# leospeidel/Colate

Hardware: NVIDIA B200
Metric: pair_site_evals_per_s (higher is better)
Workload: dtype f64

## Files before the change

### colate_b200/csrc/kernels_em.cu

```cuda
#include <cooperative_groups.h>

#include "device.cuh"
#include "glibc_math.cuh"

#include <cstring>

namespace cg = cooperative_groups;

namespace colate {

constexpr int EM_THREADS = 416;
constexpr int EM_TASKS = 384;

__global__ void __launch_bounds__(256)
k_bootstrap(int num_blocks, const int32_t* __restrict__ weights, const double* __restrict__ blk,
            double age, const double* __restrict__ age_bin, double* __restrict__ counts, int norm_1e3)
{
  __shared__ double S[NBINS], N[NBINS], SE[NBINS], NE[NBINS], F[NBINS];
  __shared__ double s_fcount, s_normf;
  const int r = blockIdx.x;
  const int32_t* w = weights + (size_t)r * num_blocks;
  int bin_start = 0;
  while (bin_start < NBINS - 1 && age_bin[bin_start] <= age) bin_start++;
  for (int b = threadIdx.x; b < NBINS; b += blockDim.x) {
// ... 377 lines not shown
        }
        __syncthreads();
        if (tid < cw) {
          double acc = 0.0;
#pragma unroll 10
          for (int j = 0; j < n_task; j++) acc += stage[j * cw + tid];
          const int col = c0 + tid;
          for (int r = 0; r < csize; r++) {
            if (col < E) cluster.map_shared_rank(tn, r)[col] = acc;
            else if (col < 2 * E) cluster.map_shared_rank(td, r)[col - E] = acc;
            else cluster.map_shared_rank(&ll_new, r)[0] = acc;
          }
        }
        __syncthreads();
      }
      cluster.sync();
      if (tid == 0) { prev_s = ll_s; ll_s = ll_new; }
    } else {
      double acc = 0.0;
      int buf = 0;
      for (int col = tid + EM_THREADS; col <= 2 * E; col += EM_THREADS) (col < 2 * E ? tn[col] : ll_new) = 0.0;
      for (int i = tid; i < min(TJ, n_task) * RS; i += blockDim.x) stage[i] = __ldcg(M + i);
      __syncthreads();
      for (int j0 = 0; j0 < n_task; j0 += TJ) {
        const int nj = min(TJ, n_task - j0);
        const int j1 = j0 + TJ, nn = (j1 < n_task) ? min(TJ, n_task - j1) : 0;
        double pre[9];
        const double* src = M + (size_t)j1 * RS;
#pragma unroll
        for (int u = 0; u < 9; u++) { const int i = tid + u * EM_THREADS; pre[u] = (i < nn * RS) ? __ldcg(src + i) : 0.0; }
        if (tid <= 2 * E) {
          const double* col = stage + (size_t)buf * EM_STAGE_DOUBLES + tid;
          for (int j = 0; j < nj; j++) acc += col[(size_t)j * RS];
        }
        for (int c2 = tid + EM_THREADS; c2 <= 2 * E; c2 += EM_THREADS) {
          const double* col = stage + (size_t)buf * EM_STAGE_DOUBLES + c2;
          double& a2 = c2 < 2 * E ? tn[c2] : ll_new;
          double s = a2;
          for (int j = 0; j < nj; j++) s += col[(size_t)j * RS];
          a2 = s;
        }
        double* dst = stage + (size_t)(buf ^ 1) * EM_STAGE_DOUBLES;
#pragma unroll
        for (int u = 0; u < 9; u++) { const int i = tid + u * EM_THREADS; if (i < nn * RS) dst[i] = pre[u]; }
        __syncthreads();
        buf ^= 1;
      }
      if (tid < E) tn[tid] = acc;
      else if (tid < 2 * E) td[tid - E] = acc;
      else if (tid == 2 * E) { prev_s = ll_s; ll_s = acc; }
      if (2 * E >= EM_THREADS && tid == 2 * E % EM_THREADS) { prev_s = ll_s; ll_s = ll_new; }
    }
    __syncthreads();
    if (prof) { t1 = clock64(); tp[4] += t1 - t0; t0 = t1; }
    for (int e = tid; e < E; e += blockDim.x) {
      const double n_ = tn[e], d_ = td[e];
      double r = rate[e];
      if (n_ != 0 && d_ != 0) { r = n_ / d_; r = (r < 5e-9) ? 5e-9 : r; }
      cand[e] = r;
    }
    __syncthreads();
    for (int e = tid; e < E; e += blockDim.x) {
      int s = e;
      while (s >= 0 && tn[s] == 0) s--;
      rate[e] = (s >= 0) ? cand[s] : 0.0;
    }
    if (tid == 0 && (ll_s / prev_s > 1.0 - 1e-7) && (iter > 1000)) stop_flag = 1;
    __syncthreads();
    if (prof) { t1 = clock64(); tp[5] += t1 - t0; t0 = t1; }
    if (stop_flag) break;
  }
  if (prof && tid == 0) for (int i = 0; i < 6; i++) prof[i] = tp[i];
  if (prof && tid == 384) prof[6] = tp[1];
  if (prof && tid == 192 + 8 * crank + 1) prof[7] = tp[1];
  if (crank == 0) {
    for (int e = tid; e < E; e += blockDim.x) rates_out[(size_t)rep * E + e] = rate[e];
    if (tid == 0) { iters_out[rep] = iter; ll_out[rep] = ll_s; }
  }
}

constexpr int EMS_THREADS = 640;
constexpr int EMS_FOLD_WARPS = 12;
constexpr int EMS_TLMAX = 96;

__device__ __forceinline__ uint32_t em_smem_u32(const void* p) { return (uint32_t)__cvta_generic_to_shared(p); }
__device__ __forceinline__ uint32_t em_mapa(uint32_t saddr, int rank)
{
  uint32_t r;
  asm volatile("mapa.shared::cluster.u32 %0, %1, %2;" : "=r"(r) : "r"(saddr), "r"(rank));
  return r;
}
__device__ __forceinline__ void em_st_async(uint32_t raddr, double v, uint32_t rbar)
{
  asm volatile("st.async.weak.shared::cluster.mbarrier::complete_tx::bytes.b64 [%0], %1, [%2];" ::"r"(raddr),
               "l"(__double_as_longlong(v)), "r"(rbar) : "memory");
}
__device__ __forceinline__ void em_mbar_init(uint64_t* bar, int count)
{
  asm volatile("mbarrier.init.shared::cta.b64 [%0], %1;" ::"r"(em_smem_u32(bar)), "r"(count) : "memory");
}
__device__ __forceinline__ void em_mbar_arm(uint64_t* bar, uint32_t bytes)
{
  asm volatile("mbarrier.arrive.expect_tx.shared::cta.b64 _, [%0], %1;" ::"r"(em_smem_u32(bar)), "r"(bytes) : "memory");
}
__device__ __forceinline__ bool em_mbar_wait(uint64_t* bar, uint32_t parity)
{
  const long long t0 = clock64();
  for (;;) {
    uint32_t done;
    asm volatile(
        "{\n\t.reg .pred p;\n\t"
        "mbarrier.try_wait.parity.acquire.cluster.shared::cta.b64 p, [%1], %2;\n\t"
        "selp.u32 %0, 1, 0, p;\n\t}" : "=r"(done) : "r"(em_smem_u32(bar)), "r"(parity) : "memory");
    if (done) return true;
    if (clock64() - t0 > 4000000000ll) return false;
  }
}
__device__ __forceinline__ void named_bar_sync(int id, int n) { asm volatile("bar.sync %0, %1;" ::"r"(id), "r"(n) : "memory"); }
__device__ __forceinline__ void named_bar_arrive(int id, int n) { asm volatile("bar.arrive %0, %1;" ::"r"(id), "r"(n) : "memory"); }

__global__ void __launch_bounds__(EMS_THREADS, 1)
k_em_split(int E, const double* __restrict__ epochs, const double* __restrict__ rates_init,
           const double* __restrict__ age_bin_g, const double* __restrict__ counts, int max_iter,
           const uint64_t* __restrict__ exp_tab_g, const uint64_t* __restrict__ log_tab_g, double* scratch,
           double* __restrict__ rates_out, int32_t* __restrict__ iters_out, double* __restrict__ ll_out, long long* prof_g)
{
  cg::cluster_group cluster = cg::this_cluster();
  const int crank = (int)cluster.block_rank(), csize = (int)cluster.num_blocks();
  const int rep = blockIdx.x / csize;
  const int n_task = 2 * NBINS, ncol = 2 * E + 1, RS = 2 * E + 2;
  const int CW = (ncol + csize - 1) / csize;
  const int nbl = (NBINS + csize - 1) / csize;
  const int ntl = 2 * nbl;

  extern __shared__ double sm[];
  double* ep = sm;
  double* rate = ep + E;
  double* Lam = rate + E;
  double* A = Lam + E;
  double* B = A + E;
  double* PL = B + E;
  double* tn = PL + E + 1;
  double* td = tn + E;
  double* cand = td + E;
  double* prod = cand + E;
  double* raw = prod + E;
  double* integ_s = raw + (size_t)ntl * E * 2;
  double* colbuf = integ_s + (size_t)ntl * E;
  uint64_t* etab = (uint64_t*)(colbuf + (size_t)n_task * CW);
  uint64_t* ltab = etab + 256;
  __shared__ int stop_flag;
  __shared__ double ll_s, prev_s, ll_new;
  __shared__ __align__(8) uint64_t bar_rows, bar_tot;
  __shared__ double h_t[EMS_TLMAX], h_cnt[EMS_TLMAX], h_nc[EMS_TLMAX], h_numt[EMS_TLMAX], h_dent[EMS_TLMAX], h_logl[EMS_TLMAX];
  __shared__ int h_et[EMS_TLMAX], h_good[EMS_TLMAX];

  const int tid = threadIdx.x, warp = tid >> 5, lane = tid & 31;
  const uint32_t magicE = E > 1 ? 0xffffffffu / (uint32_t)E + 1u : 0u, magicCW = CW > 1 ? 0xffffffffu / (uint32_t)CW + 1u : 0u;
  auto divE = [&](int i) { return magicE ? (int)__umulhi((uint32_t)i, magicE) : i; };
  auto divCW = [&](int c) { return magicCW ? (int)__umulhi((uint32_t)c, magicCW) : c; };
  for (int e = tid; e < E; e += blockDim.x) { ep[e] = epochs[e]; rate[e] = rates_init[e]; }
  for (int i = tid; i < 256; i += blockDim.x) { etab[i] = exp_tab_g[i]; ltab[i] = log_tab_g[i]; }
  if (tid == 0) {
    stop_flag = 0; ll_s = neg_inf();
    em_mbar_init(&bar_rows, 1); em_mbar_init(&bar_tot, 1);
    asm volatile("fence.mbarrier_init.release.cluster;" ::: "memory");
  }
  const int n_active = __syncthreads_count(tid < n_task && counts[(size_t)rep * 2 * NBINS + tid] > 0);
  const int my_cw = max(0, min(ncol, crank * CW + CW) - crank * CW);
  const uint32_t bytes_rows = (uint32_t)n_active * my_cw * 8, bytes_tot = (uint32_t)ncol * 8;
  const uint32_t colbuf_s = em_smem_u32(colbuf), tn_s = em_smem_u32(tn), td_s = em_smem_u32(td), ll_sa = em_smem_u32(&ll_new);
  const uint32_t bar_rows_s = em_smem_u32(&bar_rows), bar_tot_s = em_smem_u32(&bar_tot);
  if (tid < ntl) {
    const int b = (tid >> 1) * csize + crank, type = tid & 1;
    double t = 0.0, cnt = 0.0;
    if (b < NBINS) { t = age_bin_g[b]; cnt = counts[(size_t)rep * 2 * NBINS + (type ? NBINS : 0) + b]; }
    h_t[tid] = t;
    h_cnt[tid] = cnt > 0 ? cnt : 0.0;
    h_et[tid] = tint_k(E, ep, t) - 1;
    h_good[tid] = 0; h_nc[tid] = 0.0; h_numt[tid] = 0.0; h_dent[tid] = 0.0; h_logl[tid] = 0.0;
  }
  for (int i = tid; i < n_task * CW; i += blockDim.x) colbuf[i] = 0.0;
  EmCtx c{E, ep, rate, A, B, Lam, glm::Tables{etab, ltab}};
  long long* prof = prof_g ? prof_g + (size_t)blockIdx.x * 16 : nullptr;
  long long tp[16] = {0, 0, 0, 0, 0, 0, 0, 0, 0, 0, 0, 0, 0, 0, 0, 0};
  cluster.sync();

  int iter = 0;
  for (; iter < max_iter; iter++) {
    long long t0 = prof ? clock64() : 0, t1;
    if (tid == 0) { em_mbar_arm(&bar_rows, bytes_rows); em_mbar_arm(&bar_tot, bytes_tot); }
    for (int e = tid + 1; e < E; e += blockDim.x) prod[e] = rate[e - 1] * (ep[e] - ep[e - 1]);
    __syncthreads();
    for (int e = tid; e < E; e += blockDim.x) {
      double l = 0.0;
      for (int i = 1; i <= e; i++) l = l + prod[i];
      Lam[e] = l;
    }
    __syncthreads();
    const int ft0 = (E + 31) & ~31;
    if (tid < E) em_A(E, ep, rate, Lam, tid, A, c.T);
    else if (tid >= ft0 && tid < ft0 + nbl && h_cnt[2 * (tid - ft0) + 1] > 0) {
      const int l = 2 * (tid - ft0) + 1, et = h_et[l], k = et + 1;
      const double t = h_t[l], r = rate[et];
      const double c1 = Lam[et] + r * (t - ep[et]);
      const double c2 = c1 + r * (t - t);
      double num_t;
      if (et != E - 1) {
        const double c3 = c2 + r * (ep[k] - t);
        num_t = (r > 0) ? lme(-c2, -c3, c.T) : neg_inf();
      } else num_t = -c2;
      h_numt[l] = num_t;
    }
    __syncthreads();
    if (prof) { t1 = clock64(); tp[0] += t1 - t0; t0 = t1; }
    if (warp < EMS_FOLD_WARPS) {
      const int fpw = (nbl + EMS_FOLD_WARPS - 1) / EMS_FOLD_WARPS;
      const int f = warp * fpw + lane, l = 2 * f + 1;
      if (lane < fpw && f < nbl && h_cnt[l] > 0) {
        double nc = h_numt[l];
        const int et = h_et[l];
        if (et != E - 1) {
          double v = A[et + 1];
          for (int e = et + 1; e < E; e++) {
            const double vn = A[min(e + 1, E - 1)];
            nc = lse(nc, v, c.T);
            v = vn;
          }
        }
        const bool good = !bad(nc);
        h_nc[l] = nc; h_good[l] = good ? 1 : 0; h_logl[l] = h_cnt[l] * (good ? nc : 0.0);
      }
    } else if (warp == EMS_FOLD_WARPS) {
      if (lane == 0) {
        double nc = A[0], v = A[min(1, E - 1)];
        PL[0] = 1.0;
        PL[1] = nc;
        for (int e = 1; e < E; e++) {
          const double vn = A[min(e + 1, E - 1)];
          if (nc == 1.0) nc = v; else nc = lse(nc, v, c.T);
          PL[e + 1] = nc;
          v = vn;
        }
      }
      named_bar_sync(1, EMS_THREADS - EMS_FOLD_WARPS * 32);
      for (int j = lane; j < nbl; j += 32) {
        const int l = 2 * j;
        if (h_cnt[l] > 0) {
          const double pl = PL[h_et[l]], num_t = h_numt[l];
          const double nc = (pl == 1.0) ? num_t : lse(pl, num_t, c.T);
          const bool good = !bad(nc);
          h_nc[l] = nc; h_good[l] = good ? 1 : 0; h_logl[l] = h_cnt[l] * (good ? nc : 0.0);
        }
      }
    } else {
      const int q = tid - (EMS_FOLD_WARPS + 1) * 32;
      if (q < E) em_B(E, ep, rate, Lam, q, B, c.T);
      else if (q < E + nbl) {
        const int l = 2 * (q - E) + 1;
        if (h_cnt[l] > 0) {
          const int et = h_et[l], k = et + 1;
          const double t = h_t[l], r = rate[et], inv = 1.0 / r;
          const double c1 = Lam[et] + r * (t - ep[et]);
          const double c2 = c1 + r * (t - t);
          double den_t;
          if (et != E - 1) {
            const double c3 = c2 + r * (ep[k] - t);
            den_t = (r > 0) ? glm::log((t + inv) - (ep[k] + inv) * glm::exp(-c3 + c2, c.T), c.T) - c2 : neg_inf();
          } else den_t = glm::log(t + inv, c.T) - c2;
          h_dent[l] = den_t;
        }
      } else if (q < E + 2 * nbl) {
        const int l = 2 * (q - E - nbl);
        if (h_cnt[l] > 0) {
          double num_t, den_t;
          shared_special(c, h_t[l], h_et[l], num_t, den_t);
          h_numt[l] = num_t; h_dent[l] = den_t;
        }
      }
      named_bar_arrive(1, EMS_THREADS - EMS_FOLD_WARPS * 32);
    }
    __syncthreads();
    if (prof) { t1 = clock64(); tp[1] += t1 - t0; t0 = t1; }
    auto raw_term = [&](int i, int which) {
      const int l = divE(i), e = i - l * E, et = h_et[l];
      const bool sh = (l & 1) == 0;
      const int lim = (E - 1 < et + 1) ? E - 1 : et + 1;
      const bool need = h_good[l] && (sh ? (e < lim || (e == E - 1 && et == E - 1)) : (e >= et));
      const bool own = sh ? !(e < et) : (e == et);
      if (need) {
        const double x = (which == 0 ? (own ? h_numt[l] : A[e]) : (own ? h_dent[l] : B[e])) - h_nc[l];
        raw[2 * i + which] = exp_fast(x, c.T);
      }
    };
    for (int i = tid; i < ntl * E; i += blockDim.x) raw_term(i, 0);
    __syncthreads();
    if (prof) { t1 = clock64(); tp[2] += t1 - t0; t0 = t1; }
    const int iw = ((ntl + 31) >> 5) * 32;
    if (tid >= iw) {
      for (int i = tid - iw; i < ntl * E; i += blockDim.x - iw) raw_term(i, 1);
    } else if (tid < ntl && h_good[tid]) {
      const int et = h_et[tid];
      const int lo = (tid & 1) ? et : 0;
      const int hi = (tid & 1) ? E - 1 : ((E - 1 < et + 1) ? E - 1 : et + 1);
      double integ = 1.0;
      const double* __restrict__ rw = raw + (size_t)tid * E * 2;
      double* __restrict__ out = integ_s + tid * E;
      for (int e0 = 0; e0 < E; e0 += 8) {
        double nb[8];
#pragma unroll
        for (int u = 0; u < 8; u++) nb[u] = (e0 + u >= lo && e0 + u < hi) ? rw[2 * (e0 + u)] : 0.0;
#pragma unroll
        for (int u = 0; u < 8; u++) {
          integ = (integ > 0.0) ? integ - nb[u] : 0.0;
          if (e0 + u < E) out[e0 + u] = integ;
        }
      }
    }
    __syncthreads();
    if (prof) { t1 = clock64(); tp[8] += t1 - t0; t0 = t1; }
    for (int i = tid; i < ntl * E; i += blockDim.x) {
      const int l = divE(i), e = i - l * E;
      const double cnt = h_cnt[l];
      if (cnt > 0) {
        const int et = h_et[l];
        double ne = 0.0, de = 0.0;
        if (h_good[l]) {
          const double integ = integ_s[i];
          if ((l & 1) == 0) {
            const int lim = (E - 1 < et + 1) ? E - 1 : et + 1;
            if (e < lim) {
              ne = raw[2 * i];
              de = raw[2 * i + 1];
              de += -ep[e] * ne + (ep[e + 1] - ep[e]) * integ;
              if (de < 0.0) de = 0.0;
            } else if (e == E - 1 && et == E - 1) {
              ne = raw[2 * i];
              de = raw[2 * i + 1];
              de -= ep[e] * ne;
              if (de < 0.0) de = 0.0;
            }
          } else {
            if (e < et) {
              de = ep[e + 1] - ep[e];
            } else {
              ne = raw[2 * i];
              if (e < E - 1) {
                de = raw[2 * i + 1];
                de += -ep[e] * ne + (ep[e + 1] - ep[e]) * integ;
              } else {
                de = raw[2 * i + 1];
                de -= ep[e] * ne;
              }
              if (de < 0.0) de = 0.0;
            }
          }
        }
        const int tk = 2 * ((l >> 1) * csize + crank) + (l & 1);
        const int r1 = divCW(e), r2 = divCW(E + e);
        em_st_async(em_mapa(colbuf_s, r1) + 8u * (tk * CW + (e - r1 * CW)), cnt * ne, em_mapa(bar_rows_s, r1));
        em_st_async(em_mapa(colbuf_s, r2) + 8u * (tk * CW + (E + e - r2 * CW)), cnt * de, em_mapa(bar_rows_s, r2));
      }
    }
    if (tid < ntl && h_cnt[tid] > 0) {
      const int tk = 2 * ((tid >> 1) * csize + crank) + (tid & 1), r = (2 * E) / CW;
      em_st_async(em_mapa(colbuf_s, r) + 8u * (tk * CW + (2 * E - r * CW)), h_logl[tid], em_mapa(bar_rows_s, r));
    }
    if (prof) { t1 = clock64(); tp[6] += t1 - t0; t0 = t1; }
    if (warp == 0 && !em_mbar_wait(&bar_rows, iter & 1)) stop_flag = 2;
    __syncthreads();
    if (prof) { t1 = clock64(); tp[3] += t1 - t0; t0 = t1; }
    {
      const int cbeg = crank * CW, cw = max(0, min(ncol, cbeg + CW) - cbeg);
      if (prof) { t1 = clock64(); tp[7] += t1 - t0; t0 = t1; }
      if (tid < cw) {
        double acc = 0.0;
#pragma unroll 10
        for (int j = 0; j < n_task; j++) acc += colbuf[j * CW + tid];
        prod[tid] = acc;
      }
      __syncthreads();
      for (int i = tid; i < cw * csize; i += blockDim.x) {
        const int r = i / cw, cc = i - r * cw, col = cbeg + cc;
        const double acc = prod[cc];
        const uint32_t dst = col < E ? tn_s + 8u * col : col < 2 * E ? td_s + 8u * (col - E) : ll_sa;
        em_st_async(em_mapa(dst, r), acc, em_mapa(bar_tot_s, r));
      }
      if (warp == 0 && !em_mbar_wait(&bar_tot, iter & 1)) stop_flag = 2;
      __syncthreads();
      if (tid == 0) { prev_s = ll_s; ll_s = ll_new; }
    }
    __syncthreads();
    if (prof) { t1 = clock64(); tp[4] += t1 - t0; t0 = t1; }
    for (int e = tid; e < E; e += blockDim.x) {
      const double n_ = tn[e], d_ = td[e];
      double r = rate[e];
      if (n_ != 0 && d_ != 0) { r = n_ / d_; r = (r < 5e-9) ? 5e-9 : r; }
      cand[e] = r;
    }
    __syncthreads();
    for (int e = tid; e < E; e += blockDim.x) {
      int s = e;
      while (s >= 0 && tn[s] == 0) s--;
      rate[e] = (s >= 0) ? cand[s] : 0.0;
    }
    if (tid == 0 && stop_flag == 0 && (ll_s / prev_s > 1.0 - 1e-7) && (iter > 1000)) stop_flag = 1;
    __syncthreads();
    if (prof) { t1 = clock64(); tp[5] += t1 - t0; t0 = t1; }
    if (stop_flag) break;
  }
  if (prof && tid == 0) for (int i = 0; i < 16; i++) prof[i] = tp[i];
  cluster.sync();
  if (crank == 0) {
    for (int e = tid; e < E; e += blockDim.x) rates_out[(size_t)rep * E + e] = rate[e];
    if (tid == 0) { iters_out[rep] = iter; ll_out[rep] = ll_s; }
  }
  if (stop_flag == 2 && tid == 0) iters_out[rep] = -1;
}

constexpr int EMC_THREADS = 640;
constexpr int EMC_FOLD_WARPS = 6;
constexpr int EMC_NT = 384;

struct EmcTask { int lo, hi, off, et; };

__host__ __device__ inline int emc_block(int type, int et, int E)
{
  const int n = type ? E - et : ((E - 1 < et + 1 ? E - 1 : et + 1) + (et == E - 1 ? 1 : 0));
  return type ? (n + 1) & ~1 : n | 1;
}

template <bool kGrids>
__device__ __forceinline__ void em_cta_body(int E, int n_pairs_cap, const double* __restrict__ epochs, const double* __restrict__ rates_init,
                                            const double* __restrict__ age_bin_g, const double* __restrict__ counts, int max_iter,
                                            const uint64_t* __restrict__ exp_tab_g, const uint64_t* __restrict__ log_tab_g,
                                            double* __restrict__ rates_out, int32_t* __restrict__ iters_out, double* __restrict__ ll_out,
                                            long long* prof_g, const int32_t* __restrict__ grid_of, const int4* __restrict__ grid_info,
                                            int E_out)
{
  const int rep = blockIdx.x;
  if (kGrids) {
    const int4 g = grid_info[grid_of[rep]];
    E = g.x; n_pairs_cap = g.z;
    epochs += g.y; rates_init += g.y;
  }
  extern __shared__ double sm[];
  double* ep = sm;
  double* rate = ep + E;
  double* Lam = rate + E;
  double* A = Lam + E;
  double* B = A + E;
  double* PL = B + E;
  double* tn = PL + E + 1;
  double* td = tn + E;
  double* cand = td + E;
  double* prod = cand + E;
  double* wz = prod + E;
  double* h_t = sm + ((11 * E + 2 + 1) & ~1);
  double* h_cnt = h_t + 192;
  double* h_cg = h_cnt + EMC_NT;
  double* h_nc = h_cg + EMC_NT;
  double* h_numt = h_nc + EMC_NT;
  double* h_dent = h_numt + EMC_NT;
  double* h_logl = h_dent + EMC_NT;
  double* valN = h_logl + EMC_NT;
  double* valD = valN + n_pairs_cap;
  uint64_t* etab = (uint64_t*)(valD + n_pairs_cap);
  uint64_t* ltab = etab + 256;
  EmcTask* task = (EmcTask*)(ltab + 256);
  int4* binrec = (int4*)(task + EMC_NT);
  int* h_good = (int*)(binrec + 192);
  uint16_t* pair_task = (uint16_t*)(h_good + EMC_NT);
  __shared__ int stop_flag, n_pairs_s;
  __shared__ double ll_s, prev_s;

  const int tid = threadIdx.x, warp = tid >> 5, lane = tid & 31;
  const int n_task = 2 * NBINS;
  for (int e = tid; e < E; e += blockDim.x) { ep[e] = epochs[e]; rate[e] = rates_init[e]; }
  for (int i = tid; i < 256; i += blockDim.x) { etab[i] = exp_tab_g[i]; ltab[i] = log_tab_g[i]; }
  if (tid == 0) { stop_flag = 0; ll_s = neg_inf(); }
  __syncthreads();
  for (int e = tid; e <= E; e += blockDim.x) wz[e] = (e >= 1 && e < E) ? ep[e] - ep[e - 1] : 0.0;
  if (tid < EMC_NT) {
    const int b = tid >> 1, type = tid & 1;
    double t = 0.0, cnt = 0.0;
    int et = 0;
    if (b < NBINS) {
      t = age_bin_g[b];
      cnt = counts[(size_t)rep * 2 * NBINS + (type ? NBINS : 0) + b];
      et = tint_k(E, ep, t) - 1;
      if (type == 0) h_t[b] = t;
    }
    h_cnt[tid] = cnt > 0 ? cnt : 0.0;
    h_cg[tid] = 0.0;
    h_good[tid] = 0; h_nc[tid] = 0.0; h_numt[tid] = 0.0; h_dent[tid] = 0.0; h_logl[tid] = 0.0;
    EmcTask k;
// ... 302 lines not shown
                       const uint64_t* __restrict__ log_tab_g, double* __restrict__ y)
{
  glm::Tables T{exp_tab_g, log_tab_g};
  for (int i = blockIdx.x * blockDim.x + threadIdx.x; i < n; i += gridDim.x * blockDim.x)
    y[i] = which == 0 ? glm::exp(x[i], T) : which == 1 ? glm::log(x[i], T) : glm::log1p(x[i]);
}

__global__ void k_test_em_prims(int which, int n, const double* __restrict__ a, const double* __restrict__ b,
                                const uint64_t* __restrict__ exp_tab_g, const uint64_t* __restrict__ log_tab_g, double* __restrict__ y,
                                int32_t* __restrict__ ok)
{
  glm::Tables T{exp_tab_g, log_tab_g};
  for (int i = blockIdx.x * blockDim.x + threadIdx.x; i < n; i += gridDim.x * blockDim.x) {
    const double x = a[i], x2 = b[i];
    double r = 0.0;
    bool k = true;
    if (which == 0) { r = glm::exp_main(x, T); k = glm::exp_is_main(x); }
    else if (which == 1) { r = glm::log1p_k0(x); k = glm::log1p_is_k0(x); }
    else if (which == 2) { r = glm::log1p_wide(x); k = glm::log1p_wide_ok(x); }
    else if (which == 3) r = glm::div_midrange(x, x2);
    else if (which == 4 || which == 5) {
      const double d = -fabs(x - x2), e = glm::exp_main(d, T);
      r = which == 4 ? lse(x, x2, T) : lse_wide(x, x2, T);
      k = !bad(x) & !bad(x2) & glm::exp_is_main(d) & (which == 4 ? glm::log1p_is_k0(e) : glm::log1p_wide_ok(e));
    } else {
      const double d = x2 - x, e = -glm::exp_main(d, T);
      r = lme(x, x2, T);
      k = !bad(x) & !bad(x2) & !(x < x2) & glm::exp_is_main(d) & glm::log1p_is_k0(e);
    }
    y[i] = r;
    ok[i] = k ? 1 : 0;
  }
}

int ensure_libm_tables(colate_handle* h)
{
  if (h->libm_tab.p) return 0;
  CK(h->libm_tab.ensure(512 * 8));
  CK(cudaMemcpyAsync(h->libm_tab.p, glm::hEXP_TAB, 256 * 8, cudaMemcpyHostToDevice, h->stream));
  CK(cudaMemcpyAsync(h->libm_tab.as<uint64_t>() + 256, glm::hLOG_TAB, 256 * 8, cudaMemcpyHostToDevice, h->stream));
  CK(cudaStreamSynchronize(h->stream));
  return 0;
}

int run_bootstrap(colate_handle* h, int R, int num_blocks, const double* block_stats_dev, double age)
{
  k_bootstrap<<<R, 256, 0, h->stream>>>(num_blocks, h->d_weights.as<int32_t>(), block_stats_dev, age,
                                        h->d_agebin.as<double>(), h->d_counts.as<double>(), h->opt_norm_1e3 ? 1 : 0);
  h->launches += 1;
  CK(cudaGetLastError());
  return 0;
}

bool em_cta_fits(const colate_handle* h, int E, const double* epochs_host, int* n_pairs_cap, size_t* smem)
{
  const double* ab = h->h_agebin;
  int cap = 0;
  for (int b = 0; b < NBINS; b++) {
    int k = E;
    for (int e = 0; e < E; e++) if (ab[b] < epochs_host[e]) { k = e; break; }
    cap += emc_block(0, k - 1, E) + emc_block(1, k - 1, E);
  }
  *n_pairs_cap = cap;
  *smem = sizeof(double) * ((size_t)11 * E + 4 + 192 + 6 * EMC_NT + 2 * (size_t)cap) + 512 * 8 + EMC_NT * (sizeof(EmcTask) + 4) + 192 * 16 +
          (size_t)cap * 2 + 32;
  return *smem <= 225 * 1024 && ((E + 31) & ~31) + NBINS <= EMC_THREADS;
}

int run_em(colate_handle* h, int R, int E, int max_iter, const double* epochs_host, cudaStream_t stream)
{
  int rc = ensure_libm_tables(h);
  if (rc) return rc;
  int csize = 1;
  if (const char* e = getenv("COLATE_EM_CLUSTER")) csize = atoi(e);
  else {
    const int sms = h->sm_count;
    while (csize < 8 && R * csize * 2 <= sms) csize *= 2;
    if (csize == 8 && R * 16 * 2 <= sms) csize = 16;
    if (csize < 8) csize = 1;
  }
  if (csize != 1 && csize != 2 && csize != 4 && csize != 8 && csize != 16) csize = 1;
  auto split_fits = [&](int cs, size_t* bytes) {
    const int nbl = (NBINS + cs - 1) / cs, ntl = 2 * nbl, CW = (2 * E + 1 + cs - 1) / cs;
    *bytes = sizeof(double) * ((size_t)10 * E + 1 + (size_t)ntl * E * 3 + (size_t)2 * NBINS * CW) + 512 * 8;
    return cs >= 8 && ntl <= EMS_TLMAX && *bytes <= 200 * 1024 && !getenv("COLATE_EM_NOSPLIT") &&
           E + 2 * nbl <= EMS_THREADS - (EMS_FOLD_WARPS + 1) * 32 && ((E + 31) & ~31) + nbl <= EMS_THREADS;
  };
  size_t smem_split = 0;
  bool split = split_fits(csize, &smem_split);
  if (!split && csize > 8) { csize = 8; split = split_fits(csize, &smem_split); }
  bool cta = false;
  size_t smem_cta = 0;
  int n_pairs_cap = 0;
  const char* force = getenv("COLATE_EM_KERNEL");
  if ((!split && csize == 1 && !(force && !strcmp(force, "task"))) || (force && !strcmp(force, "cta"))) {
    cta = em_cta_fits(h, E, epochs_host, &n_pairs_cap, &smem_cta);
    if (cta) { split = false; csize = 1; }
  }
  const size_t smem = cta ? smem_cta : split ? smem_split : sizeof(double) * ((size_t)10 * E + 1 + 2 * EM_STAGE_DOUBLES) + 512 * 8;
  if (cta) CK(cudaFuncSetAttribute(k_em_cta, cudaFuncAttributeMaxDynamicSharedMemorySize, (int)smem));
  else if (split) {
    CK(cudaFuncSetAttribute(k_em_split, cudaFuncAttributeMaxDynamicSharedMemorySize, (int)smem));
    if (csize > 8) CK(cudaFuncSetAttribute(k_em_split, cudaFuncAttributeNonPortableClusterSizeAllowed, 1));
  }
  else CK(cudaFuncSetAttribute(k_em, cudaFuncAttributeMaxDynamicSharedMemorySize, (int)std::max<size_t>(smem, 1024)));
  if (!cta) CK(h->d_em_scratch.ensure((size_t)R * 2 * (2 * E + 2) * EM_TASKS * 8 + 1024));
  long long* prof = nullptr;
  if (getenv("COLATE_EM_PROF")) {
    CK(h->d_prof.ensure((size_t)R * csize * 40 * 8));
    CK(cudaMemsetAsync(h->d_prof.p, 0, (size_t)R * csize * 40 * 8, stream));
    prof = h->d_prof.as<long long>();
  }
  h->em_kernel = cta ? 2 : split ? 1 : 0;
  h->em_csize = csize;
  cudaLaunchConfig_t cfg = {};
  cfg.gridDim = dim3(R * csize);
  cfg.blockDim = dim3(cta ? EMC_THREADS : split ? EMS_THREADS : EM_THREADS);
  cfg.dynamicSmemBytes = smem;
  cfg.stream = stream;
  cudaLaunchAttribute at[1];
  at[0].id = cudaLaunchAttributeClusterDimension;
  at[0].val.clusterDim.x = csize; at[0].val.clusterDim.y = 1; at[0].val.clusterDim.z = 1;
  cfg.attrs = at;
  cfg.numAttrs = 1;
  const uint64_t* tabs = h->libm_tab.as<uint64_t>();
  if (cta)
    CK(cudaLaunchKernelEx(&cfg, k_em_cta, E, n_pairs_cap, (const double*)h->d_epochs.as<double>(), (const double*)h->d_rates.as<double>(),
                          (const double*)h->d_agebin.as<double>(), (const double*)h->d_counts.as<double>(), max_iter, tabs, tabs + 256,
                          h->d_rates.as<double>() + E, h->d_iters.as<int32_t>(), h->d_ll.as<double>(), prof));
  else
  CK(cudaLaunchKernelEx(&cfg, split ? k_em_split : k_em, E, (const double*)h->d_epochs.as<double>(), (const double*)h->d_rates.as<double>(),
                        (const double*)h->d_agebin.as<double>(), (const double*)h->d_counts.as<double>(), max_iter, tabs, tabs + 256,
                        h->d_em_scratch.as<double>(), h->d_rates.as<double>() + E, h->d_iters.as<int32_t>(), h->d_ll.as<double>(), prof));
  h->launches += 1;
  CK(cudaGetLastError());
  if (prof) {
    if (cta) {
      long long q[16];
      CK(cudaMemcpyAsync(q, prof, 128, cudaMemcpyDeviceToHost, stream));
      CK(cudaStreamSynchronize(stream));
      for (int w = 0; w < 2; w++)
        fprintf(stderr, "[k_em_cta prof, replicate 0 thread %d, cycles between its arrivals at the phase barriers] P0 %lld | P1 folds %lld | heads %lld | P2 exps %lld | P3 integ %lld | P4 column sums %lld | M-step %lld\n",
                w ? 639 : 0, q[8 * w], q[8 * w + 1], q[8 * w + 2], q[8 * w + 3], q[8 * w + 4], q[8 * w + 5], q[8 * w + 6]);
      return 0;
    }
    const int ps = split ? 16 : 8;
    std::vector<long long> hp((size_t)ps * csize);
    CK(cudaMemcpyAsync(hp.data(), prof, (size_t)ps * 8 * csize, cudaMemcpyDeviceToHost, stream));
    CK(cudaStreamSynchronize(stream));
    for (int r = 0; r < csize; r++) {
      const long long* q = hp.data() + (size_t)ps * r;
      if (split)
        fprintf(stderr, "[k_em_split prof, replicate 0 CTA %d thread 0, cycles] A + first terms %lld | folds %lld | raw exps %lld | integ %lld | rows out %lld | cluster.sync %lld | gather %lld | sums + broadcast + sync %lld | M-step %lld\n",
                r, q[0], q[1], q[2], q[8], q[6], q[3], q[7], q[4] - q[7], q[5]);
      else
        fprintf(stderr, "[k_em prof, replicate 0 CTA %d thread 0, cycles] AB %lld | folds + tasks %lld (prefix-chain thread %lld, a not-shared task %lld) | cluster.sync %lld | column sums %lld | M-step %lld (csize %d)\n",
                r, q[0], q[1], q[6], q[7], q[3], q[4], q[5], csize);
    }
  }
  return 0;
}

int run_em_grids(colate_handle* h, int R, const int32_t* grid_of_dev, const int* grid_info_dev, int E_out, size_t smem, int max_iter,
                 cudaStream_t stream)
{
  int rc = ensure_libm_tables(h);
  if (rc) return rc;
  CK(cudaFuncSetAttribute(k_em_cta_grids, cudaFuncAttributeMaxDynamicSharedMemorySize, (int)smem));
  const uint64_t* tabs = h->libm_tab.as<uint64_t>();
  k_em_cta_grids<<<R, EMC_THREADS, smem, stream>>>(grid_of_dev, (const int4*)grid_info_dev, h->d_epochs.as<double>(), h->d_rates.as<double>(),
                                                   h->d_agebin.as<double>(), h->d_counts.as<double>(), max_iter, tabs, tabs + 256, E_out,
                                                   h->d_gr_rates.as<double>(), h->d_iters.as<int32_t>(), h->d_ll.as<double>());
  h->launches += 1;
  h->em_kernel = 2;
  h->em_csize = 1;
  CK(cudaGetLastError());
  return 0;
}

int run_estep(colate_handle* h, int shared, int E, int n_t)
{
  int rc = ensure_libm_tables(h);
  if (rc) return rc;
  const size_t smem = sizeof(double) * (6 * E + 1);
  CK(cudaFuncSetAttribute(k_estep, cudaFuncAttributeMaxDynamicSharedMemorySize, (int)smem));
  double* base = h->d_tmp.as<double>();
  const uint64_t* tabs = h->libm_tab.as<uint64_t>();
  k_estep<<<1, 256, smem, h->stream>>>(shared, E, h->d_epochs.as<double>(), h->d_rates.as<double>(), n_t, base, tabs, tabs + 256,
                                       base + n_t, base + n_t + (size_t)n_t * E, base + n_t + 2 * (size_t)n_t * E);
  CK(cudaGetLastError());
  return 0;
}

int run_libm(colate_handle* h, int which, int n, const double* x_host, double* y_host)
{
  int rc = ensure_libm_tables(h);
  if (rc) return rc;
  CK(h->d_tmp.ensure((size_t)n * 16));
  double* d = h->d_tmp.as<double>();
  const uint64_t* tabs = h->libm_tab.as<uint64_t>();
  CK(cudaMemcpyAsync(d, x_host, (size_t)n * 8, cudaMemcpyHostToDevice, h->stream));
  k_libm<<<296, 256, 0, h->stream>>>(which, n, d, tabs, tabs + 256, d + n);
  CK(cudaMemcpyAsync(y_host, d + n, (size_t)n * 8, cudaMemcpyDeviceToHost, h->stream));
  CK(cudaStreamSynchronize(h->stream));
  return 0;
}

int run_test_em_prims(colate_handle* h, int which, int n, const double* a_host, const double* b_host, double* y_host, int32_t* ok_host)
{
  int rc = ensure_libm_tables(h);
  if (rc) return rc;
  CK(h->d_tmp.ensure((size_t)n * 28));
  double* d = h->d_tmp.as<double>();
  int32_t* dok = (int32_t*)(d + 3 * (size_t)n);
  const uint64_t* tabs = h->libm_tab.as<uint64_t>();
  CK(cudaMemcpyAsync(d, a_host, (size_t)n * 8, cudaMemcpyHostToDevice, h->stream));
  if (b_host) CK(cudaMemcpyAsync(d + n, b_host, (size_t)n * 8, cudaMemcpyHostToDevice, h->stream));
  else CK(cudaMemsetAsync(d + n, 0, (size_t)n * 8, h->stream));
  k_test_em_prims<<<296, 256, 0, h->stream>>>(which, n, d, d + n, tabs, tabs + 256, d + 2 * (size_t)n, dok);
  CK(cudaGetLastError());
  CK(cudaMemcpyAsync(y_host, d + 2 * (size_t)n, (size_t)n * 8, cudaMemcpyDeviceToHost, h->stream));
  CK(cudaMemcpyAsync(ok_host, dok, (size_t)n * 4, cudaMemcpyDeviceToHost, h->stream));
  CK(cudaStreamSynchronize(h->stream));
  return 0;
}

}
```

Baseline: 443.7 million.

## Restructure split EM iteration into per-warp finish pipeline with fewer block barriers

Each EM iteration in the cluster-split kernel now runs as a warp-level pipeline. Fold warps and the prefix-chain warp hand off through mbarriers and named barriers round by round. Each warp then computes its task's exps, integral and row pushes itself in per-warp scratch, replacing several block-wide phases separated by __syncthreads. The rate array is double-buffered, and the cumulative hazard is recomputed inline, which removes the prod/Lam prefix pass and its syncs. Column sums and the broadcast are handled by a single warp, and the M-step is folded into one pass. Applicability is restricted to cluster sizes 8/16 with E and CW limits. The main risk is the added serial per-warp work and more complex barrier accounting.

```diff
diff --git a/colate_b200/csrc/kernels_em.cu b/colate_b200/csrc/kernels_em.cu
--- a/colate_b200/csrc/kernels_em.cu
+++ b/colate_b200/csrc/kernels_em.cu
@@ -483,6 +483,8 @@
 constexpr int EMS_THREADS = 640;
 constexpr int EMS_FOLD_WARPS = 12;
 constexpr int EMS_TLMAX = 96;
+constexpr int EMS_WARPS = EMS_THREADS / 32;
+constexpr int EMS_SH_WARPS = EMS_WARPS - EMS_FOLD_WARPS - 1;
 
 __device__ __forceinline__ uint32_t em_smem_u32(const void* p) { return (uint32_t)__cvta_generic_to_shared(p); }
 __device__ __forceinline__ uint32_t em_mapa(uint32_t saddr, int rank)
@@ -499,6 +501,10 @@
 __device__ __forceinline__ void em_mbar_init(uint64_t* bar, int count)
 {
   asm volatile("mbarrier.init.shared::cta.b64 [%0], %1;" ::"r"(em_smem_u32(bar)), "r"(count) : "memory");
+}
+__device__ __forceinline__ void em_mbar_arrive(uint64_t* bar)
+{
+  asm volatile("mbarrier.arrive.shared::cta.b64 _, [%0];" ::"r"(em_smem_u32(bar)) : "memory");
 }
 __device__ __forceinline__ void em_mbar_arm(uint64_t* bar, uint32_t bytes)
 {
@@ -536,40 +542,39 @@
 
   extern __shared__ double sm[];
   double* ep = sm;
-  double* rate = ep + E;
-  double* Lam = rate + E;
+  double* rbuf = ep + E;
+  double* Lam = rbuf + 2 * E;
   double* A = Lam + E;
   double* B = A + E;
   double* PL = B + E;
   double* tn = PL + E + 1;
   double* td = tn + E;
-  double* cand = td + E;
-  double* prod = cand + E;
-  double* raw = prod + E;
-  double* integ_s = raw + (size_t)ntl * E * 2;
-  double* colbuf = integ_s + (size_t)ntl * E;
+  double* wsc = td + E;
+  double* colbuf = wsc + (size_t)(EMS_WARPS - 1) * 3 * E;
   uint64_t* etab = (uint64_t*)(colbuf + (size_t)n_task * CW);
   uint64_t* ltab = etab + 256;
   __shared__ int stop_flag;
+  __shared__ int rnd_et[(EMS_TLMAX / 2 + EMS_SH_WARPS - 1) / EMS_SH_WARPS];
   __shared__ double ll_s, prev_s, ll_new;
   __shared__ __align__(8) uint64_t bar_rows, bar_tot;
-  __shared__ double h_t[EMS_TLMAX], h_cnt[EMS_TLMAX], h_nc[EMS_TLMAX], h_numt[EMS_TLMAX], h_dent[EMS_TLMAX], h_logl[EMS_TLMAX];
-  __shared__ int h_et[EMS_TLMAX], h_good[EMS_TLMAX];
+  __shared__ __align__(8) uint64_t bar_b;
+  __shared__ double h_t[EMS_TLMAX], h_cnt[EMS_TLMAX], h_numt[EMS_TLMAX], h_dent[EMS_TLMAX];
+  __shared__ int h_et[EMS_TLMAX];
 
   const int tid = threadIdx.x, warp = tid >> 5, lane = tid & 31;
-  const uint32_t magicE = E > 1 ? 0xffffffffu / (uint32_t)E + 1u : 0u, magicCW = CW > 1 ? 0xffffffffu / (uint32_t)CW + 1u : 0u;
-  auto divE = [&](int i) { return magicE ? (int)__umulhi((uint32_t)i, magicE) : i; };
+  const uint32_t magicCW = CW > 1 ? 0xffffffffu / (uint32_t)CW + 1u : 0u;
   auto divCW = [&](int c) { return magicCW ? (int)__umulhi((uint32_t)c, magicCW) : c; };
-  for (int e = tid; e < E; e += blockDim.x) { ep[e] = epochs[e]; rate[e] = rates_init[e]; }
+  for (int e = tid; e < E; e += blockDim.x) { ep[e] = epochs[e]; rbuf[e] = rates_init[e]; }
   for (int i = tid; i < 256; i += blockDim.x) { etab[i] = exp_tab_g[i]; ltab[i] = log_tab_g[i]; }
   if (tid == 0) {
-    stop_flag = 0; ll_s = neg_inf();
-    em_mbar_init(&bar_rows, 1); em_mbar_init(&bar_tot, 1);
+    stop_flag = 0; ll_s = neg_inf(); PL[0] = 1.0;
+    em_mbar_init(&bar_rows, 1); em_mbar_init(&bar_tot, 1); em_mbar_init(&bar_b, EMS_SH_WARPS * 32);
     asm volatile("fence.mbarrier_init.release.cluster;" ::: "memory");
   }
   const int n_active = __syncthreads_count(tid < n_task && counts[(size_t)rep * 2 * NBINS + tid] > 0);
   const int my_cw = max(0, min(ncol, crank * CW + CW) - crank * CW);
-  const uint32_t bytes_rows = (uint32_t)n_active * my_cw * 8, bytes_tot = (uint32_t)ncol * 8;
+  __shared__ uint32_t bytes_rows, bytes_tot;
+  if (tid == 0) { bytes_rows = (uint32_t)n_active * my_cw * 8; bytes_tot = (uint32_t)ncol * 8; }
   const uint32_t colbuf_s = em_smem_u32(colbuf), tn_s = em_smem_u32(tn), td_s = em_smem_u32(td), ll_sa = em_smem_u32(&ll_new);
   const uint32_t bar_rows_s = em_smem_u32(&bar_rows), bar_tot_s = em_smem_u32(&bar_tot);
   if (tid < ntl) {
@@ -579,84 +584,180 @@
     h_t[tid] = t;
     h_cnt[tid] = cnt > 0 ? cnt : 0.0;
     h_et[tid] = tint_k(E, ep, t) - 1;
-    h_good[tid] = 0; h_nc[tid] = 0.0; h_numt[tid] = 0.0; h_dent[tid] = 0.0; h_logl[tid] = 0.0;
+    h_numt[tid] = 0.0; h_dent[tid] = 0.0;
   }
   for (int i = tid; i < n_task * CW; i += blockDim.x) colbuf[i] = 0.0;
-  EmCtx c{E, ep, rate, A, B, Lam, glm::Tables{etab, ltab}};
+  const glm::Tables T{etab, ltab};
   long long* prof = prof_g ? prof_g + (size_t)blockIdx.x * 16 : nullptr;
-  long long tp[16] = {0, 0, 0, 0, 0, 0, 0, 0, 0, 0, 0, 0, 0, 0, 0, 0};
+  __shared__ long long tp[10];
+  if (tid < 10) tp[tid] = 0;
   cluster.sync();
+  const int n_rounds = (nbl + EMS_SH_WARPS - 1) / EMS_SH_WARPS;
+  if (tid == 0) {
+    int m = 0;
+    for (int k = 0; k < n_rounds; k++) {
+      for (int j = k * EMS_SH_WARPS; j < min(nbl, (k + 1) * EMS_SH_WARPS); j++) m = max(m, h_et[2 * j]);
+      rnd_et[k] = m;
+    }
+  }
+
+  auto finish = [&](int l, int et, double cnt, double nc, double num_t, double den_t) {
+    const bool sh = (l & 1) == 0, good = !bad(nc);
+    const int lim = (E - 1 < et + 1) ? E - 1 : et + 1;
+    double* s_ne = wsc + (size_t)(warp < EMS_FOLD_WARPS ? warp : warp - 1) * 3 * E;
+    double* s_de = s_ne + E;
+    double* s_in = s_de + E;
+    __syncwarp();
+    int f = E;
+    if (good) {
+      for (int e = lane; e < E; e += 32) {
+        const bool need = sh ? (e < lim || (e == E - 1 && et == E - 1)) : (e >= et);
+        const bool own = sh ? !(e < et) : (e == et);
+        if (need) {
+          s_ne[e] = exp_fast((own ? num_t : A[e]) - nc, T);
+          s_de[e] = exp_fast((own ? den_t : B[e]) - nc, T);
+        }
+      }
+      __syncwarp();
+      if (lane == 0) {
+        const int lo = sh ? 0 : et, hi = sh ? lim : E - 1;
+        double integ = 1.0;
+        for (int e0 = 0; e0 < E; e0 += 8) {
+          double nb[8];
+#pragma unroll
+          for (int u = 0; u < 8; u++) nb[u] = (e0 + u >= lo && e0 + u < hi) ? s_ne[e0 + u] : 0.0;
+#pragma unroll
+          for (int u = 0; u < 8; u++) {
+            integ = integ - nb[u];
+            if (e0 + u < E) s_in[e0 + u] = integ;
+            if (!(integ > 0.0) && e0 + u < f) f = e0 + u;
+          }
+        }
+      }
+      f = __shfl_sync(0xffffffffu, f, 0);
+      __syncwarp();
+    }
+    const int tk = 2 * ((l >> 1) * csize + crank) + (l & 1);
+    for (int e = lane; e < E; e += 32) {
+      double ne = 0.0, de = 0.0;
+      if (good) {
+        const double integ = (e > f) ? 0.0 : s_in[e];
+        if (sh) {
+          if (e < lim) {
+            ne = s_ne[e];
+            de = s_de[e];
+            de += -ep[e] * ne + (ep[e + 1] - ep[e]) * integ;
+            if (de < 0.0) de = 0.0;
+          } else if (e == E - 1 && et == E - 1) {
+            ne = s_ne[e];
+            de = s_de[e];
+            de -= ep[e] * ne;
+            if (de < 0.0) de = 0.0;
+          }
+        } else {
+          if (e < et) {
+            de = ep[e + 1] - ep[e];
+          } else {
+            ne = s_ne[e];
+            if (e < E - 1) {
+              de = s_de[e];
+              de += -ep[e] * ne + (ep[e + 1] - ep[e]) * integ;
+            } else {
+              de = s_de[e];
+              de -= ep[e] * ne;
+            }
+            if (de < 0.0) de = 0.0;
+          }
+        }
+      }
+      const int r1 = divCW(e), r2 = divCW(E + e);
+      em_st_async(em_mapa(colbuf_s, r1) + 8u * (tk * CW + (e - r1 * CW)), cnt * ne, em_mapa(bar_rows_s, r1));
+      em_st_async(em_mapa(colbuf_s, r2) + 8u * (tk * CW + (E + e - r2 * CW)), cnt * de, em_mapa(bar_rows_s, r2));
+    }
+    if (lane == 0) {
+      const int r = (2 * E) / CW;
+      em_st_async(em_mapa(colbuf_s, r) + 8u * (tk * CW + (2 * E - r * CW)), cnt * (good ? nc : 0.0), em_mapa(bar_rows_s, r));
+    }
+  };
 
   int iter = 0;
   for (; iter < max_iter; iter++) {
     long long t0 = prof ? clock64() : 0, t1;
+    double* const rate = rbuf + (size_t)(iter & 1) * E;
+    const EmCtx c{E, ep, rate, A, B, Lam, T};
     if (tid == 0) { em_mbar_arm(&bar_rows, bytes_rows); em_mbar_arm(&bar_tot, bytes_tot); }
-    for (int e = tid + 1; e < E; e += blockDim.x) prod[e] = rate[e - 1] * (ep[e] - ep[e - 1]);
-    __syncthreads();
-    for (int e = tid; e < E; e += blockDim.x) {
+    auto cumhaz = [&](int e) {
       double l = 0.0;
-      for (int i = 1; i <= e; i++) l = l + prod[i];
-      Lam[e] = l;
-    }
-    __syncthreads();
+      for (int i = 1; i <= e; i++) l = l + rate[i - 1] * (ep[i] - ep[i - 1]);
+      return l;
+    };
     const int ft0 = (E + 31) & ~31;
-    if (tid < E) em_A(E, ep, rate, Lam, tid, A, c.T);
-    else if (tid >= ft0 && tid < ft0 + nbl && h_cnt[2 * (tid - ft0) + 1] > 0) {
+    if (tid < E) {
+      const int e = tid;
+      const double l0 = cumhaz(e), r = rate[e];
+      Lam[e] = l0;
+      if (e < E - 1) {
+        const double l1 = l0 + r * (ep[e + 1] - ep[e]);
+        const double tb = ep[e], te = ep[e + 1];
+        A[e] = (r > 0 && te != 0 && te - tb > 0) ? lme(-l0, -l1, T) : neg_inf();
+      } else A[e] = (r > 0) ? -l0 : neg_inf();
+    } else if (tid >= ft0 && tid < ft0 + nbl && h_cnt[2 * (tid - ft0) + 1] > 0) {
       const int l = 2 * (tid - ft0) + 1, et = h_et[l], k = et + 1;
       const double t = h_t[l], r = rate[et];
-      const double c1 = Lam[et] + r * (t - ep[et]);
+      const double c1 = cumhaz(et) + r * (t - ep[et]);
       const double c2 = c1 + r * (t - t);
       double num_t;
       if (et != E - 1) {
         const double c3 = c2 + r * (ep[k] - t);
-        num_t = (r > 0) ? lme(-c2, -c3, c.T) : neg_inf();
+        num_t = (r > 0) ? lme(-c2, -c3, T) : neg_inf();
       } else num_t = -c2;
       h_numt[l] = num_t;
     }
     __syncthreads();
-    if (prof) { t1 = clock64(); tp[0] += t1 - t0; t0 = t1; }
+    if (prof) { t1 = clock64(); if (tid == 0) tp[0] += t1 - t0; t0 = t1; }
     if (warp < EMS_FOLD_WARPS) {
       const int fpw = (nbl + EMS_FOLD_WARPS - 1) / EMS_FOLD_WARPS;
       const int f = warp * fpw + lane, l = 2 * f + 1;
+      double nc = 0.0;
       if (lane < fpw && f < nbl && h_cnt[l] > 0) {
-        double nc = h_numt[l];
+        nc = h_numt[l];
         const int et = h_et[l];
         if (et != E - 1) {
           double v = A[et + 1];
           for (int e = et + 1; e < E; e++) {
             const double vn = A[min(e + 1, E - 1)];
-            nc = lse(nc, v, c.T);
+            nc = lse(nc, v, T);
             v = vn;
           }
         }
-        const bool good = !bad(nc);
-        h_nc[l] = nc; h_good[l] = good ? 1 : 0; h_logl[l] = h_cnt[l] * (good ? nc : 0.0);
-      }
+        if (prof && tid == 0) tp[7] += E - 1 - et;
+      }
+      if (prof && tid == 0) { t1 = clock64(); tp[1] += t1 - t0; t0 = t1; }
+      if (!em_mbar_wait(&bar_b, iter & 1)) stop_flag = 2;
+      if (prof && tid == 0) { t1 = clock64(); tp[9] += t1 - t0; t0 = t1; }
+      for (int q = 0; q < fpw; q++) {
+        const int fq = warp * fpw + q, lq = 2 * fq + 1;
+        const double ncq = __shfl_sync(0xffffffffu, nc, q);
+        if (fq < nbl && h_cnt[lq] > 0) finish(lq, h_et[lq], h_cnt[lq], ncq, h_numt[lq], h_dent[lq]);
+      }
+      if (prof && tid == 0) { t1 = clock64(); tp[2] += t1 - t0; t0 = t1; }
     } else if (warp == EMS_FOLD_WARPS) {
-      if (lane == 0) {
-        double nc = A[0], v = A[min(1, E - 1)];
-        PL[0] = 1.0;
-        PL[1] = nc;
-        for (int e = 1; e < E; e++) {
+      double nc = 1.0, v = A[0];
+      int e = 0;
+      for (int k = 0; k < n_rounds; k++) {
+        const int upto = rnd_et[k];
+        for (; e < upto; e++) {
           const double vn = A[min(e + 1, E - 1)];
-          if (nc == 1.0) nc = v; else nc = lse(nc, v, c.T);
-          PL[e + 1] = nc;
+          if (nc == 1.0) nc = v; else nc = lse(nc, v, T);
+          if (lane == 0) PL[e + 1] = nc;
           v = vn;
         }
-      }
-      named_bar_sync(1, EMS_THREADS - EMS_FOLD_WARPS * 32);
-      for (int j = lane; j < nbl; j += 32) {
-        const int l = 2 * j;
-        if (h_cnt[l] > 0) {
-          const double pl = PL[h_et[l]], num_t = h_numt[l];
-          const double nc = (pl == 1.0) ? num_t : lse(pl, num_t, c.T);
-          const bool good = !bad(nc);
-          h_nc[l] = nc; h_good[l] = good ? 1 : 0; h_logl[l] = h_cnt[l] * (good ? nc : 0.0);
-        }
-      }
+        named_bar_arrive(3 + k, 32 * (1 + min(EMS_SH_WARPS, nbl - k * EMS_SH_WARPS)));
+      }
+      if (prof && lane == 0) tp[8] += clock64() - t0;
     } else {
       const int q = tid - (EMS_FOLD_WARPS + 1) * 32;
-      if (q < E) em_B(E, ep, rate, Lam, q, B, c.T);
+      if (q < E) em_B(E, ep, rate, Lam, q, B, T);
       else if (q < E + nbl) {
         const int l = 2 * (q - E) + 1;
         if (h_cnt[l] > 0) {
@@ -667,8 +768,8 @@
           double den_t;
           if (et != E - 1) {
             const double c3 = c2 + r * (ep[k] - t);
-            den_t = (r > 0) ? glm::log((t + inv) - (ep[k] + inv) * glm::exp(-c3 + c2, c.T), c.T) - c2 : neg_inf();
-          } else den_t = glm::log(t + inv, c.T) - c2;
+            den_t = (r > 0) ? glm::log((t + inv) - (ep[k] + inv) * glm::exp(-c3 + c2, T), T) - c2 : neg_inf();
+          } else den_t = glm::log(t + inv, T) - c2;
           h_dent[l] = den_t;
         }
       } else if (q < E + 2 * nbl) {
@@ -679,140 +780,60 @@
           h_numt[l] = num_t; h_dent[l] = den_t;
         }
       }
-      named_bar_arrive(1, EMS_THREADS - EMS_FOLD_WARPS * 32);
-    }
-    __syncthreads();
-    if (prof) { t1 = clock64(); tp[1] += t1 - t0; t0 = t1; }
-    auto raw_term = [&](int i, int which) {
-      const int l = divE(i), e = i - l * E, et = h_et[l];
-      const bool sh = (l & 1) == 0;
-      const int lim = (E - 1 < et + 1) ? E - 1 : et + 1;
-      const bool need = h_good[l] && (sh ? (e < lim || (e == E - 1 && et == E - 1)) : (e >= et));
-      const bool own = sh ? !(e < et) : (e == et);
-      if (need) {
-        const double x = (which == 0 ? (own ? h_numt[l] : A[e]) : (own ? h_dent[l] : B[e])) - h_nc[l];
-        raw[2 * i + which] = exp_fast(x, c.T);
-      }
-    };
-    for (int i = tid; i < ntl * E; i += blockDim.x) raw_term(i, 0);
-    __syncthreads();
-    if (prof) { t1 = clock64(); tp[2] += t1 - t0; t0 = t1; }
-    const int iw = ((ntl + 31) >> 5) * 32;
-    if (tid >= iw) {
-      for (int i = tid - iw; i < ntl * E; i += blockDim.x - iw) raw_term(i, 1);
-    } else if (tid < ntl && h_good[tid]) {
-      const int et = h_et[tid];
-      const int lo = (tid & 1) ? et : 0;
-      const int hi = (tid & 1) ? E - 1 : ((E - 1 < et + 1) ? E - 1 : et + 1);
-      double integ = 1.0;
-      const double* __restrict__ rw = raw + (size_t)tid * E * 2;
-      double* __restrict__ out = integ_s + tid * E;
-      for (int e0 = 0; e0 < E; e0 += 8) {
-        double nb[8];
-#pragma unroll
-        for (int u = 0; u < 8; u++) nb[u] = (e0 + u >= lo && e0 + u < hi) ? rw[2 * (e0 + u)] : 0.0;
-#pragma unroll
-        for (int u = 0; u < 8; u++) {
-          integ = (integ > 0.0) ? integ - nb[u] : 0.0;
-          if (e0 + u < E) out[e0 + u] = integ;
-        }
-      }
-    }
-    __syncthreads();
-    if (prof) { t1 = clock64(); tp[8] += t1 - t0; t0 = t1; }
-    for (int i = tid; i < ntl * E; i += blockDim.x) {
-      const int l = divE(i), e = i - l * E;
-      const double cnt = h_cnt[l];
-      if (cnt > 0) {
-        const int et = h_et[l];
-        double ne = 0.0, de = 0.0;
-        if (h_good[l]) {
-          const double integ = integ_s[i];
-          if ((l & 1) == 0) {
-            const int lim = (E - 1 < et + 1) ? E - 1 : et + 1;
-            if (e < lim) {
-              ne = raw[2 * i];
-              de = raw[2 * i + 1];
-              de += -ep[e] * ne + (ep[e + 1] - ep[e]) * integ;
-              if (de < 0.0) de = 0.0;
-            } else if (e == E - 1 && et == E - 1) {
-              ne = raw[2 * i];
-              de = raw[2 * i + 1];
-              de -= ep[e] * ne;
-              if (de < 0.0) de = 0.0;
-            }
-          } else {
-            if (e < et) {
-              de = ep[e + 1] - ep[e];
-            } else {
-              ne = raw[2 * i];
-              if (e < E - 1) {
-                de = raw[2 * i + 1];
-                de += -ep[e] * ne + (ep[e + 1] - ep[e]) * integ;
-              } else {
-                de = raw[2 * i + 1];
-                de -= ep[e] * ne;
-              }
-              if (de < 0.0) de = 0.0;
-            }
-          }
-        }
-        const int tk = 2 * ((l >> 1) * csize + crank) + (l & 1);
-        const int r1 = divCW(e), r2 = divCW(E + e);
-        em_st_async(em_mapa(colbuf_s, r1) + 8u * (tk * CW + (e - r1 * CW)), cnt * ne, em_mapa(bar_rows_s, r1));
-        em_st_async(em_mapa(colbuf_s, r2) + 8u * (tk * CW + (E + e - r2 * CW)), cnt * de, em_mapa(bar_rows_s, r2));
-      }
-    }
-    if (tid < ntl && h_cnt[tid] > 0) {
-      const int tk = 2 * ((tid >> 1) * csize + crank) + (tid & 1), r = (2 * E) / CW;
-      em_st_async(em_mapa(colbuf_s, r) + 8u * (tk * CW + (2 * E - r * CW)), h_logl[tid], em_mapa(bar_rows_s, r));
-    }
-    if (prof) { t1 = clock64(); tp[6] += t1 - t0; t0 = t1; }
-    if (warp == 0 && !em_mbar_wait(&bar_rows, iter & 1)) stop_flag = 2;
-    __syncthreads();
-    if (prof) { t1 = clock64(); tp[3] += t1 - t0; t0 = t1; }
-    {
+      em_mbar_arrive(&bar_b);
+      named_bar_sync(1, EMS_SH_WARPS * 32);
+      for (int j = warp - (EMS_FOLD_WARPS + 1), k = 0; j < nbl; j += EMS_SH_WARPS, k++) {
+        named_bar_sync(3 + k, 32 * (1 + min(EMS_SH_WARPS, nbl - k * EMS_SH_WARPS)));
+        const int l = 2 * j;
+        if (h_cnt[l] > 0) {
+          const int et = h_et[l];
+          const double pl = PL[et], num_t = h_numt[l];
+          const double nc = (pl == 1.0) ? num_t : lse(pl, num_t, T);
+          finish(l, et, h_cnt[l], nc, num_t, h_dent[l]);
+        }
+      }
+    }
+    if (warp == 0) {
+      if (!em_mbar_wait(&bar_rows, iter & 1)) stop_flag = 2;
+      if (prof && tid == 0) { t1 = clock64(); tp[3] += t1 - t0; t0 = t1; }
       const int cbeg = crank * CW, cw = max(0, min(ncol, cbeg + CW) - cbeg);
-      if (prof) { t1 = clock64(); tp[7] += t1 - t0; t0 = t1; }
-      if (tid < cw) {
+      if (lane < cw) {
         double acc = 0.0;
 #pragma unroll 10
-        for (int j = 0; j < n_task; j++) acc += colbuf[j * CW + tid];
-        prod[tid] = acc;
-      }
-      __syncthreads();
-      for (int i = tid; i < cw * csize; i += blockDim.x) {
-        const int r = i / cw, cc = i - r * cw, col = cbeg + cc;
-        const double acc = prod[cc];
+        for (int j = 0; j < n_task; j++) acc += colbuf[j * CW + lane];
+        const int col = cbeg + lane;
         const uint32_t dst = col < E ? tn_s + 8u * col : col < 2 * E ? td_s + 8u * (col - E) : ll_sa;
-        em_st_async(em_mapa(dst, r), acc, em_mapa(bar_tot_s, r));
-      }
-      if (warp == 0 && !em_mbar_wait(&bar_tot, iter & 1)) stop_flag = 2;
-      __syncthreads();
-      if (tid == 0) { prev_s = ll_s; ll_s = ll_new; }
-    }
-    __syncthreads();
-    if (prof) { t1 = clock64(); tp[4] += t1 - t0; t0 = t1; }
-    for (int e = tid; e < E; e += blockDim.x) {
-      const double n_ = tn[e], d_ = td[e];
-      double r = rate[e];
-      if (n_ != 0 && d_ != 0) { r = n_ / d_; r = (r < 5e-9) ? 5e-9 : r; }
-      cand[e] = r;
-    }
-    __syncthreads();
-    for (int e = tid; e < E; e += blockDim.x) {
-      int s = e;
+        for (int r = 0; r < csize; r++) em_st_async(em_mapa(dst, r), acc, em_mapa(bar_tot_s, r));
+      }
+      if (prof && tid == 0) { t1 = clock64(); tp[4] += t1 - t0; t0 = t1; }
+    }
+    double* rate_next = rbuf + (size_t)((iter + 1) & 1) * E;
+    bool quit = false;
+    if (tid < E) {
+      if (!em_mbar_wait(&bar_tot, iter & 1)) stop_flag = 2;
+      if (prof && tid == 0) { t1 = clock64(); tp[5] += t1 - t0; t0 = t1; }
+      int s = tid;
       while (s >= 0 && tn[s] == 0) s--;
-      rate[e] = (s >= 0) ? cand[s] : 0.0;
-    }
-    if (tid == 0 && stop_flag == 0 && (ll_s / prev_s > 1.0 - 1e-7) && (iter > 1000)) stop_flag = 1;
-    __syncthreads();
-    if (prof) { t1 = clock64(); tp[5] += t1 - t0; t0 = t1; }
-    if (stop_flag) break;
-  }
-  if (prof && tid == 0) for (int i = 0; i < 16; i++) prof[i] = tp[i];
+      double r = 0.0;
+      if (s >= 0) {
+        const double n_ = tn[s], d_ = td[s];
+        r = rate[s];
+        if (n_ != 0 && d_ != 0) { r = n_ / d_; r = (r < 5e-9) ? 5e-9 : r; }
+      }
+      rate_next[tid] = r;
+      if (tid == 0) { prev_s = ll_s; ll_s = ll_new; quit = (ll_s / prev_s > 1.0 - 1e-7) && (iter > 1000); }
+    }
+    quit = __syncthreads_or(quit) || stop_flag;
+    if (prof && tid == 0) { t1 = clock64(); tp[6] += t1 - t0; t0 = t1; }
+    if (quit) break;
+  }
+  if (prof && tid == 0) {
+    for (int i = 0; i < 10; i++) prof[i] = tp[i];
+    prof[10] = iter + (iter < max_iter ? 1 : 0);
+  }
   cluster.sync();
   if (crank == 0) {
+    const double* rate = rbuf + (size_t)((iter + (iter < max_iter ? 1 : 0)) & 1) * E;
     for (int e = tid; e < E; e += blockDim.x) rates_out[(size_t)rep * E + e] = rate[e];
     if (tid == 0) { iters_out[rep] = iter; ll_out[rep] = ll_s; }
   }
@@ -1281,9 +1302,10 @@
   if (csize != 1 && csize != 2 && csize != 4 && csize != 8 && csize != 16) csize = 1;
   auto split_fits = [&](int cs, size_t* bytes) {
     const int nbl = (NBINS + cs - 1) / cs, ntl = 2 * nbl, CW = (2 * E + 1 + cs - 1) / cs;
-    *bytes = sizeof(double) * ((size_t)10 * E + 1 + (size_t)ntl * E * 3 + (size_t)2 * NBINS * CW) + 512 * 8;
-    return cs >= 8 && ntl <= EMS_TLMAX && *bytes <= 200 * 1024 && !getenv("COLATE_EM_NOSPLIT") &&
-           E + 2 * nbl <= EMS_THREADS - (EMS_FOLD_WARPS + 1) * 32 && ((E + 31) & ~31) + nbl <= EMS_THREADS;
+    *bytes = sizeof(double) * ((size_t)9 * E + 1 + (size_t)(EMS_WARPS - 1) * 3 * E + (size_t)2 * NBINS * CW) + 512 * 8;
+    return (cs == 16 || cs == 8) && E <= (cs == 16 ? 193 : 100) && !getenv("COLATE_EM_NOSPLIT") && ntl <= EMS_TLMAX &&
+           CW <= 32 && *bytes <= 200 * 1024 && E + 2 * nbl <= EMS_THREADS - (EMS_FOLD_WARPS + 1) * 32 &&
+           ((E + 31) & ~31) + nbl <= EMS_THREADS;
   };
   size_t smem_split = 0;
   bool split = split_fits(csize, &smem_split);
@@ -1349,9 +1371,18 @@
     CK(cudaStreamSynchronize(stream));
     for (int r = 0; r < csize; r++) {
       const long long* q = hp.data() + (size_t)ps * r;
-      if (split)
-        fprintf(stderr, "[k_em_split prof, replicate 0 CTA %d thread 0, cycles] A + first terms %lld | folds %lld | raw exps %lld | integ %lld | rows out %lld | cluster.sync %lld | gather %lld | sums + broadcast + sync %lld | M-step %lld\n",
-                r, q[0], q[1], q[2], q[8], q[6], q[3], q[7], q[4] - q[7], q[5]);
+      if (split) {
+        const double n = q[10] > 0 ? (double)q[10] : 1.0;
+        double at[8];
+        at[0] = 0.0;
+        const int ord[7] = {0, 1, 9, 2, 3, 4, 5};
+        for (int i = 0; i < 7; i++) at[i + 1] = at[i] + q[ord[i]] / n;
+        const double len = at[7] + q[6] / n;
+        fprintf(stderr, "[k_em_split prof, replicate 0 CTA %d warp 0 (its longest not-shared fold), cycles after the iteration's start, "
+                "mean of %lld iterations] fold start %.0f | fold end %.0f (%.0f per step) | B_ep in %.0f | own tail pushed %.0f | all rows landed %.0f | "
+                "sums done %.0f | totals landed %.0f | next iteration %.0f | next fold start %.0f | prefix chain ends %.0f\n",
+                r, q[10], at[1], at[2], q[7] ? (double)q[1] / q[7] : 0.0, at[3], at[4], at[5], at[6], at[7], len, len + at[1], at[1] + q[8] / n);
+      }
       else
         fprintf(stderr, "[k_em prof, replicate 0 CTA %d thread 0, cycles] AB %lld | folds + tasks %lld (prefix-chain thread %lld, a not-shared task %lld) | cluster.sync %lld | column sums %lld | M-step %lld (csize %d)\n",
                 r, q[0], q[1], q[6], q[7], q[3], q[4], q[5], csize);
```

Measured after the change: 459.7 million, median of 6. 3.6% higher.
